# SpacewaIker/python-raytracer

Hardware: AMD Instinct MI355X
Metric: Mrays/sec + frame ms, TwoSpheresPlane 1920×1080 @1/2/4/8 GPUs (higher is better)
Workload: dtype fp32 vectors + fp64 scalars (reference numerics); 1 GPU; TwoSpheresPlane 1920x1080 1spp (primary + shadow rays); width=1920, height=1080, spp=1, parallelism=single GPU

## Files before the change

### python-raytracer_amd/csrc/rtx_api.hip

```cpp
#include <hip/hip_runtime.h>
#include <hip/hiprtc.h>

#include <algorithm>
#include <chrono>
#include <cmath>
#include <cstdio>
#include <cstring>
#include <dirent.h>
#include <fstream>
#include <functional>
#include <future>
#include <list>
#include <map>
#include <numeric>
#include <mutex>
#include <sstream>
#include <string>
#include <sys/stat.h>
#include <unistd.h>
#include <vector>

#include "../../include/rtx.h"
#include "rtx_kernels.h"
#include "rtx_bins.h"
// ... 19 lines not shown
    return code;
}

#define RTX_HIP(call)                                                                     \
    do {                                                                                  \
        hipError_t e_ = (call);                                                           \
        if (e_ != hipSuccess)                                                             \
            return fail(RTX_ERR_HIP, std::string(#call ": ") + hipGetErrorString(e_));    \
    } while (0)

enum Opt {
    OPT_SPLIT, OPT_SPLIT_BYTES, OPT_SPLIT_RATIO, OPT_BINS, OPT_HEAVY_TILES, OPT_LENS_BINS, OPT_LGRID, OPT_DSGRID, OPT_DSGRID_MIN,
    OPT_SELF_SKIP, OPT_TILE_SCHED, OPT_XCD_MAP, OPT_TILE_BLOCK, OPT_PRIM_ORIGIN, OPT_SPP, OPT_SPP_MIN, OPT_JIT, OPT_JIT_BAKE, OPT_JIT_EXT,
    OPT_JIT_DUMP, OPT_JIT_IDLE_BAKED, OPT_JIT_DISK_BAKED, OPT_JIT_CACHE, OPT_JIT_FLAGS, OPT_JIT_ILP, OPT_JIT_ASYNC,
    OPT_DEV_BINS, OPT_CHUNK_MODE, OPT_BIN_LDS, OPT_JIT_CSG, OPT_CSG_RAYS, OPT_CSG_SHADE, OPT_SETUP_LOG, OPT_SHADOW_BINS,
    OPT_UNIFORM_HIT, OPT_RAY_TABLE, OPT_RAY_TABLE_MAX_MB, OPT_COUNT
};
struct OptDef {
    const char* name;
    double dflt;
    bool str;
};
constexpr OptDef kOpts[OPT_COUNT] = {
    {"split", 1, false},
    {"split_bytes", 2147483648.0, false},
    {"split_ratio", -1, false},
    {"bins", 1, false},
    {"heavy_tiles", 1, false},
    {"lens_bins", 1, false},
    {"lgrid", 1, false},
    {"dsgrid", 1, false},
// ... 14 lines not shown
    {"jit_cache", 0, true},
    {"jit_flags", 0, true},
    {"jit_ilp", 1, false},
    {"jit_async", 1, false},
    {"dev_bins", 1, false},
    {"chunk_mode", 3, false},
    {"bin_lds", 0, false},
    {"jit_csg", 1, false},
    {"csg_rays", 3, false},
    {"csg_shade", 0, false},
    {"setup_log", 0, false},
    {"shadow_bins", 1, false},
    {"uniform_hit", 1, false},
    {"ray_table", 1, false},
    {"ray_table_max_mb", 64, false},
};
struct OptVal {
    double v;
    std::string s;
};
std::mutex g_opt_mu;
OptVal* opt_table() {
    static OptVal* t = [] {
        static OptVal vals[OPT_COUNT];
        for (int i = 0; i < OPT_COUNT; ++i) {
            vals[i].v = kOpts[i].dflt;
            std::string env = "RTX_";
            for (const char* c = kOpts[i].name; *c; ++c) env += (char)toupper((unsigned char)*c);
            if (const char* e = getenv(env.c_str())) {
                if (kOpts[i].str) vals[i].s = e;
// ... 938 lines not shown
    std::stable_sort(order.begin(), order.end(), [&](int32_t a2, int32_t b2) { return fz[a2] < fz[b2]; });
    for (int32_t f : order)
        for (int32_t by = rects[f].r0; by <= rects[f].r1; ++by)
            for (int32_t bx = rects[f].c0; bx <= rects[f].c1; ++bx) faces[fill[(size_t)by * nbx + bx]++] = f;
    zmin.resize(faces.size());
    for (size_t q = 0; q < faces.size(); ++q) {
        float z = (float)fz[faces[q]];
        if ((double)z > fz[faces[q]]) z = std::nextafter(z, -INFINITY);
        zmin[q] = z;
    }
    mesh_bins = 1;
    return true;
}

struct SbV { double x, y, z; };
struct SbPlane { SbV n; double num, dperp0; };
struct SbObj { SbV lo, hi, ctr; double r; uint32_t bit; int32_t sphere, always, pad; };
struct SbLight { SbV v; int32_t point, pad; };
constexpr int kSbPlanes = 8, kSbObjs = 32, kSbLights = 8, kSbSeen = 8, kSbPoints = 4 * kSbPlanes + 8 * kSbSeen;
struct SbScene {
    SbV o, cu, cv, cw;
    double d, dx, dy, margin, omag;
    int32_t W, H, bins_x, bins_y, NL, n_plane, n_obs, pad;
    uint32_t all_bits, always_bits;
    SbPlane planes[kSbPlanes];
    SbObj obs[kSbObjs];
    SbLight lights[kSbLights];
};
RTX_HD SbV sb_sub(SbV a, SbV b) { return SbV{a.x - b.x, a.y - b.y, a.z - b.z}; }
RTX_HD double sb_dot(SbV a, SbV b) { return a.x * b.x + a.y * b.y + a.z * b.z; }
RTX_HD SbV sb_axpy(SbV a, double t, SbV b) { return SbV{a.x + t * b.x, a.y + t * b.y, a.z + t * b.z}; }
RTX_HD bool sb_fin(SbV a) { return __builtin_isfinite(a.x) && __builtin_isfinite(a.y) && __builtin_isfinite(a.z); }

RTX_HD bool sb_separated(const SbV* P, int n, const SbLight& Lt, const SbObj& q, double grow) {
    SbV x = P[0];
    for (int it = 0; it < 12; ++it) {
        SbV u = sb_sub(q.ctr, x);
// ... 29 lines not shown
        if (q.sphere) {
            omin = sb_dot(u, q.ctr) - (q.r + grow) * sqrt(uu);
        } else {
            omin = fmin(u.x * (q.lo.x - grow), u.x * (q.hi.x + grow)) + fmin(u.y * (q.lo.y - grow), u.y * (q.hi.y + grow)) +
                   fmin(u.z * (q.lo.z - grow), u.z * (q.hi.z + grow));
        }
        if (m < omin - 1e-9 * (fabs(m) + fabs(omin) + 1.0)) return true;
        const SbV w = sb_sub(s, x);
        const double ww = sb_dot(w, w), t = ww > 0.0 ? sb_dot(u, w) / ww : 0.0;
        if (!(t > 1e-12)) return false;
        x = sb_axpy(x, fmin(t, 1.0), w);
    }
    return false;
}

RTX_HD void sb_bin(const SbScene& S, const float* xs, const float* ys, const uint32_t* objmask, int32_t bx, int32_t by,
                   uint32_t* out) {
    for (int32_t l = 0; l < S.NL; ++l) out[l] = S.all_bits;
    const int32_t c0 = 8 * bx, c1 = (8 * bx + 8 < S.W ? 8 * bx + 8 : S.W) - 1;
    const int32_t r0 = 8 * by, r1 = (8 * by + 8 < S.H ? 8 * by + 8 : S.H) - 1;
    const double px = 2.0 * S.margin * S.dx, py = 2.0 * S.margin * S.dy;
    const double xl = (double)xs[c0] - px, xh = (double)xs[c1] + px;
    const double yl = (double)ys[S.H - 1 - r1] - py, yh = (double)ys[S.H - 1 - r0] + py;
    if (!(xl < xh && yl < yh)) return;
    SbV dir[4];
    for (int q = 0; q < 4; ++q) {
        const double x = (q & 1) ? xh : xl, y = (q & 2) ? yh : yl;
        const SbV d{x * S.cu.x + y * S.cv.x - S.d * S.cw.x, x * S.cu.y + y * S.cv.y - S.d * S.cw.y,
                    x * S.cu.z + y * S.cv.z - S.d * S.cw.z};
        const double dd = sqrt(sb_dot(d, d));
        if (!(dd > 0.0) || !__builtin_isfinite(dd)) return;
        dir[q] = SbV{d.x / dd, d.y / dd, d.z / dd};
    }
    SbV P[kSbPoints];
    int np = 0;
    double rho = 0.0;
    for (int32_t k = 0; k < S.n_plane; ++k) {
        const SbPlane& pl = S.planes[k];
        const double sg = pl.num > 0.0 ? 1.0 : -1.0;
        double g[4], gmin = INFINITY, gmax = -INFINITY;
        for (int q = 0; q < 4; ++q) {
            g[q] = sg * sb_dot(dir[q], pl.n);
            gmin = fmin(gmin, g[q]);
            gmax = fmax(gmax, g[q]);
        }
        if (gmax <= 0.0) continue;
        if (!(gmin >= 1e-3)) return;
        double mp = 0.0;
        for (int q = 0; q < 4; ++q) {
            const SbV p = sb_axpy(S.o, fabs(pl.num) / g[q], dir[q]);
            P[np++] = p;
            mp = fmax(mp, fabs(p.x) + fabs(p.y) + fabs(p.z));
        }
        rho = fmax(rho, (pl.dperp0 + 0x1p-18 * mp) / gmin + 0x1p-20 * mp);
    }
    const uint32_t om = objmask[(int64_t)by * S.bins_x + bx];
    if (om) {
        const SbV mid{dir[0].x + dir[1].x + dir[2].x + dir[3].x, dir[0].y + dir[1].y + dir[2].y + dir[3].y,
                      dir[0].z + dir[1].z + dir[2].z + dir[3].z};
        const double mm = sqrt(sb_dot(mid, mid));
        double cosa = 1.0;
        for (int q = 0; q < 4; ++q) cosa = fmin(cosa, sb_dot(mid, dir[q]) / mm);
        if (!(cosa > 0.1)) return;
        int seen = 0;
        for (int32_t i = 0; i < S.n_obs; ++i) {
            const SbObj& q = S.obs[i];
            if (!(om & q.bit)) continue;
            if (++seen > kSbSeen) return;
            const double ov[3] = {S.o.x, S.o.y, S.o.z}, lo[3] = {q.lo.x, q.lo.y, q.lo.z}, hi[3] = {q.hi.x, q.hi.y, q.hi.z};
            double n2 = 0.0, f2 = 0.0;
            for (int a = 0; a < 3; ++a) {
// ... 17 lines not shown
        if (np == 0) {
            out[l] = S.always_bits;
            continue;
        }
        uint32_t m = S.all_bits;
        for (int32_t i = 0; i < S.n_obs; ++i) {
            const SbObj& q = S.obs[i];
            if (q.always || (om & q.bit)) continue;
            double dmax = 0.0;
            for (int j = 0; j < np; ++j) dmax = fmax(dmax, sb_dot(sb_sub(P[j], q.ctr), sb_sub(P[j], q.ctr)));
            const double grow = S.margin * ((q.sphere ? 0x1p-8 : 0x1p-10) * (sqrt(dmax) + q.r) + rho);
            if (sb_separated(P, np, S.lights[l], q, grow)) m &= ~q.bit;
        }
        out[l] = m | S.always_bits;
    }
}

__global__ __launch_bounds__(64) void k_shadow_bins(const SbScene* __restrict__ S, const float* __restrict__ xs,
                                                     const float* __restrict__ ys, const uint32_t* __restrict__ objmask,
                                                     uint32_t* __restrict__ out) {
    const int32_t b = (int32_t)(blockIdx.x * 64 + threadIdx.x);
    if (b >= S->bins_x * S->bins_y) return;
    sb_bin(*S, xs, ys, objmask, b % S->bins_x, b / S->bins_x, out + (int64_t)b * S->NL);
}

bool shadow_bins_scene(const HostScene& H, const rtx_camera_desc* c, int32_t bins_x, double margin, SbScene& S) {
    auto ldd = [](const float* p) { return SbV{(double)p[0], (double)p[1], (double)p[2]}; };
    auto amax = [](SbV a) { return std::max(std::fabs(a.x), std::max(std::fabs(a.y), std::fabs(a.z))); };
    std::memset(&S, 0, sizeof(S));
    const int32_t NL = (int32_t)H.lights.size();
    if (NL < 1 || NL > kSbLights || H.n_mesh > 0 || H.has_ext || H.n_sphere + H.n_box == 0 || H.n_sphere + H.n_box > kSbObjs ||
        H.n_plane > kSbPlanes)
        return false;
    if (c->ncols < 2 || c->height < 2 || bins_x != (c->ncols + 7) / 8) return false;
    const bool pinhole = c->n_dof == 1 && c->n_aa == 1 && c->jitter == RTX_JITTER_OFF &&
                         c->dof_origins[0] == c->position[0] && c->dof_origins[1] == c->position[1] &&
                         c->dof_origins[2] == c->position[2];
    if (!pinhole) return false;
    S.W = c->ncols; S.H = c->height; S.bins_x = bins_x; S.bins_y = (c->height + 7) / 8; S.NL = NL;
    S.o = ldd(c->aa_origins); S.cu = ldd(c->u); S.cv = ldd(c->v); S.cw = ldd(c->w);
    S.d = c->d;
    S.margin = margin;
    S.omag = amax(S.o);
    if (!sb_fin(S.o) || !sb_fin(S.cu) || !sb_fin(S.cv) || !sb_fin(S.cw) || !std::isfinite(S.d)) return false;
    for (int32_t i = 1; i < S.W; ++i) S.dx = std::max(S.dx, (double)c->xs[i] - (double)c->xs[i - 1]);
    for (int32_t j = 1; j < S.H; ++j) S.dy = std::max(S.dy, (double)c->ys[j] - (double)c->ys[j - 1]);
    if (!(S.dx > 0.0) || !(S.dy > 0.0) || !std::isfinite(S.dx + S.dy)) return false;
    double tlo = INFINITY, thi = -INFINITY;
    for (float t : camera_times(c)) {
        tlo = std::min(tlo, (double)t);
        thi = std::max(thi, (double)t);
    }
    S.n_plane = H.n_plane;
    for (int32_t k = 0; k < H.n_plane; ++k) {
        const DObj& ob = H.objs[k];
        if (ob.has_speed) return false;
        const SbV n = ldd(ob.b), p0 = ldd(ob.a);
        const double nn = std::sqrt(sb_dot(n, n));
        if (!sb_fin(n) || !sb_fin(p0) || !(nn > 0.0)) return false;
        SbPlane& pl = S.planes[k];
        pl.n = SbV{n.x / nn, n.y / nn, n.z / nn};
        pl.num = sb_dot(sb_sub(p0, S.o), pl.n);
        const double n1 = (std::fabs(n.x) + std::fabs(n.y) + std::fabs(n.z)) / nn;
        pl.dperp0 = 0x1p-19 * n1 * (std::fabs(p0.x) + std::fabs(p0.y) + std::fabs(p0.z) + std::fabs(S.o.x) + std::fabs(S.o.y) + std::fabs(S.o.z));
        if (!(std::fabs(pl.num) > 1e-9 * (1.0 + amax(p0) + S.omag))) return false;
    }
    S.n_obs = H.n_sphere + H.n_box;
    for (int32_t k = 0; k < S.n_obs; ++k) {
        const DObj& ob = H.objs[H.n_plane + k];
        SbObj& q = S.obs[k];
        q.sphere = k < H.n_sphere;
        const int32_t kk = q.sphere ? k : k - H.n_sphere;
        q.bit = 1u << ((q.sphere ? 0 : 16) + (kk & 15));
        q.always = ob.has_speed || (q.sphere ? H.n_sphere : H.n_box) > 16;
        double lo[3], hi[3];
        if (q.sphere) {
// ... 33 lines not shown
        if (!sb_fin(S.lights[l].v) || (!S.lights[l].point && !(sb_dot(S.lights[l].v, S.lights[l].v) > 0.0))) return false;
    }
    return true;
}

[[maybe_unused]] bool shadow_bins(const HostScene& H, const rtx_camera_desc* c, const std::vector<uint32_t>& objmask,
                                  int32_t bins_x, std::vector<uint32_t>& smask, double margin = 1.0) {
    smask.clear();
    SbScene S;
    if (!shadow_bins_scene(H, c, bins_x, margin, S) || objmask.size() < (size_t)S.bins_x * S.bins_y) return false;
    smask.assign((size_t)S.bins_x * S.bins_y * S.NL, S.all_bits);
    for (int32_t by = 0; by < S.bins_y; ++by)
        for (int32_t bx = 0; bx < S.bins_x; ++bx)
            sb_bin(S, c->xs, c->ys, objmask.data(), bx, by, smask.data() + ((size_t)by * S.bins_x + bx) * S.NL);
    return true;
}

bool light_grids(const HostScene& H, std::vector<DLGrid>& grids, std::vector<int32_t>& start,
                 std::vector<int32_t>& faces, std::vector<float>& d2) {
    grids.assign(H.lights.size(), DLGrid{});
    start.clear();
    faces.clear();
    d2.clear();
    if (H.n_mesh != 1) return false;
    const DObj& m = H.objs[H.n_plane + H.n_sphere + H.n_box];
    const int32_t F = m.tri_count;
    if (F < 1) return false;
    auto vert = [&](int32_t f, int k, int a) -> double {
        const DTri& T = H.tris[m.tri_begin + f];
        return k == 0 ? T.v0[a] : k == 1 ? T.v1[a] : T.v2[a];
// ... 517 lines not shown
            if (g.p) memcpy(h + g.off, g.p, g.n);
            else if (!g.dev) memset(h + g.off, 0, std::max<size_t>(g.n, 4));
        }
    }
};

struct CamTables {
    using DevFaces = std::function<int(int32_t bins_x, std::vector<int32_t>& start, int32_t* npairs, int32_t* mesh_bins)>;

    bool replay = false;
    bool pself = false;
    bool bins = false;
    bool dev_faces = false;
    bool heavy = false;
    bool sbins = false;
    bool tsched = false;
    bool po = false;
    bool rays = false;
    bool rays_dev = false;

    std::vector<float> times;
    CamStage st;
    std::vector<DBox> boxes;
    std::vector<float> pself_lim;
    std::vector<DSGrid> grids;
    std::vector<int32_t> ident, bstart, bfaces;
    std::vector<float> bz;
    std::vector<uint32_t> bmask, brmask;
    std::vector<int32_t> bheavy;
    std::vector<int2> hitems;
    SbScene sbs;
    int32_t bins_x = 0, mesh_bins = 0, dev_pairs = 0;
    int64_t tiles = 0;

    size_t host_bytes = 0;
    size_t o_xs = 0, o_ys = 0, o_dof = 0, o_aa = 0, o_times = 0, o_noise = 0, o_bounds = 0, o_pself = 0, o_dsg = 0;
    size_t o_bstart = 0, o_bfaces = 0, o_bz = 0, o_bmask = 0, o_bheavy = 0, o_hitems = 0, o_mhits = 0, o_sbs = 0;
    size_t o_bshadow = 0, o_tperm = 0, o_ttime = 0, o_kp = 0, o_rays = 0, rays_bytes = 0;

    int build(const HostScene& H, const rtx_camera_desc* c, std::vector<float> times_, const TimeTables& tr,
              const DevFaces& dev1, SetupLog& slog, bool on_device = false) {
        const size_t nsamp = (size_t)c->n_dof * c->n_aa;
        const double omax = camera_origin_bound(c);
        times = std::move(times_);
        o_xs = st.put(c->xs, sizeof(float) * c->ncols);
        o_ys = st.put(c->ys, sizeof(float) * c->height);
        o_dof = st.put(c->dof_origins, sizeof(float) * 3 * c->n_dof);
        o_aa = st.put(c->aa_origins, sizeof(float) * 3 * nsamp);
        o_times = st.put(times);
        replay = c->jitter == RTX_JITTER_REPLAY;
        if (replay) o_noise = st.put(c->noise, sizeof(float) * 3 * (size_t)c->ncols * c->height * nsamp);
        slog.mark("tables", st.size());
// ... 25 lines not shown
            o_bstart = st.put(bstart);
            if (!dev_faces) {
                o_bfaces = st.put(bfaces);
                o_bz = st.put(bz);
            }
            o_bmask = st.put(bmask);
        }
        heavy = bins && mesh_bins && !H.has_ext && opt_on(OPT_HEAVY_TILES) && heavy_chunks(bstart, bheavy, hitems);
        if (heavy) {
            o_bheavy = st.put(bheavy);
            o_hitems = st.put(hitems);
        }
        sbins = bins && opt_on(OPT_SHADOW_BINS) && (!H.has_secondary || opt(OPT_SHADOW_BINS) >= 2) && !H.has_mesh &&
                !H.has_ext && shadow_bins_scene(H, c, bins_x, 1.0, sbs);
        if (sbins) o_sbs = st.put(&sbs, sizeof(sbs));
        slog.mark("bins", st.size());
        tsched = opt_on(OPT_TILE_SCHED) && !H.has_ext && (H.has_secondary || H.has_mesh);
        int64_t nw = 0;
        if (tsched) {
            const int64_t wpb = kBlock<false> / 64;
            tiles = (int64_t)((c->ncols + 7) / 8) * ((c->height + 7) / 8);
            nw = (tiles + wpb - 1) / wpb * wpb;
            ident.resize((size_t)nw);
            std::iota(ident.begin(), ident.end(), 0);
            o_tperm = st.put(ident);
        }
        o_kp = st.put(nullptr, sizeof(KParams));
        bool boxed = true;
        for (const DObj& o : H.objs) boxed = boxed && (o.type != RTX_MESH || o.face_cull);
        rays_bytes = sizeof(float) * 3 * (size_t)ray_table_slots(c->height, c->ncols);
        rays = opt_on(OPT_RAY_TABLE) && c->n_dof == 1 && c->n_aa == 1 && c->n_times == 1 &&
               c->jitter == RTX_JITTER_OFF && !H.has_ext && ((!H.has_secondary && boxed) || opt(OPT_RAY_TABLE) == 4.0) &&
               (double)rays_bytes <= opt(OPT_RAY_TABLE_MAX_MB) * 1048576.0;
        rays_dev = rays && on_device;
        if (rays && !rays_dev) o_rays = st.put(nullptr, rays_bytes);
        host_bytes = st.size();
        if (dev_faces) {
            o_bfaces = st.put(nullptr, sizeof(int32_t) * dev_pairs, true);
            o_bz = st.put(nullptr, sizeof(float) * dev_pairs, true);
        }
        if (heavy) o_mhits = st.put(nullptr, sizeof(uint2) * 64 * hitems.size(), true);
        if (sbins) o_bshadow = st.put(nullptr, sizeof(uint32_t) * (size_t)sbs.bins_x * sbs.bins_y * sbs.NL, true);
        if (tsched) o_ttime = st.put(nullptr, sizeof(uint32_t) * nw, true);
        if (rays_dev) o_rays = st.put(nullptr, rays_bytes, true);
        slog.mark("tile schedule", st.size());
        po = c->n_dof == 1 && c->n_aa == 1 && c->jitter == RTX_JITTER_OFF && !any_moving(H) && !H.has_ext &&
             !H.has_secondary && H.n_plane <= 4 && H.n_sphere <= 16 && opt_on(OPT_PRIM_ORIGIN);
        return RTX_OK;
    }

    void bind(KParams& k, char* D, const HostScene& H, const rtx_camera_desc* c, const TimeTables& tr) const {
        k.xs = (cptr<float>)(D + o_xs);
        k.ys = (cptr<float>)(D + o_ys);
        k.dof_o = (cptr<float>)(D + o_dof);
        k.aa_o = (cptr<float>)(D + o_aa);
        k.times = (cptr<float>)(D + o_times);
        k.noise = replay ? (cptr<float>)(D + o_noise) : nullptr;
        if (!H.nodes.empty()) bind_boxes(k.S, (const DBox*)(D + o_bounds), H.nodes.size());
        if (pself) k.S.plane_self = (cptr<float>)(D + o_pself);
        if (tr.grids_on) bind_dir_grids(k.S, (const DSGrid*)(D + o_dsg), tr.cells_at());
        if (bins) {
            k.S.bin_objmask = (cptr<uint32_t>)(D + o_bmask);
            k.S.bin_rootmask = (cptr<uint32_t>)(D + o_bmask) + brmask.size();
            k.S.mesh_bins = mesh_bins;
            k.S.bin_start = (cptr<int32_t>)(D + o_bstart);
            k.S.bin_faces = (cptr<int32_t>)(D + o_bfaces);
            k.S.bin_zmin = (cptr<float>)(D + o_bz);
            k.S.bins_x = bins_x;
            k.S.bins_on = 1;
        }
        if (sbins) k.S.bin_shadow = (cptr<uint32_t>)(D + o_bshadow);
        if (heavy) {
            k.S.bin_heavy = (cptr<int32_t>)(D + o_bheavy);
            k.S.mesh_hits = reinterpret_cast<const uint2*>(D + o_mhits);
        }
        if (po) {
            const f3 o = mk(c->aa_origins[0], c->aa_origins[1], c->aa_origins[2]);
            int oi = 0;
            for (int q = 0; q < H.n_plane; ++q, ++oi) {
                const DObj& ob = H.objs[oi];
                k.po_pnum[q] = dot(sub(moved(ob, ob.a, 0.0f), o), ld3(ob.b));
            }
            for (int q = 0; q < H.n_sphere; ++q, ++oi) {
                const DObj& ob = H.objs[oi];
                const f3 oc = sub(o, moved(ob, ob.a, 0.0f));
                k.po_soc[q][0] = oc.x; k.po_soc[q][1] = oc.y; k.po_soc[q][2] = oc.z;
// ... 218 lines not shown
    if (!spp && !ext && kp.tile_time != nullptr) opts.push_back("-DRTX_TILE_SCHED=1");
    if (!spp && !ext && kp.po_valid) opts.push_back("-DRTX_PRIM_ORIGIN=1");
    if (!spp && opt_on(OPT_XCD_MAP)) opts.push_back("-DRTX_XCD_MAP=1");
    if (out8) opts.push_back("-DRTX_OUT8=1");
    if (sec && v.n_mats <= 64) opts.push_back("-DRTX_FRAME_MATBITS=6");
    if (sec && !mesh && !ext) {
        opts.push_back("-DRTX_DEFER_TIES=1");
        opts.push_back("-DRTX_HIT_T64_INLINE=1");
        opts.push_back("-DRTX_TIE_CALL=1");
        opts.push_back("-DRTX_FRAME_LDS_LEVELS=6");
        opts.push_back("-URTX_LB_WAVES");
        opts.push_back("-DRTX_LB_WAVES(MESH,SEC)=7");
    }
    opts.push_back(std::string("-DRTX_PRIMARY_BINS=") + (kp.S.bins_on ? "1" : "0"));
    if (kp.S.bins_on && kp.S.bin_shadow != nullptr) opts.push_back("-DRTX_SHADOW_BINS=1");
    if (!spp && !ext && kp.ray_dirs != nullptr && kp.n_dof * kp.n_aa * kp.n_times == 1 && kp.jitter == RTX_JITTER_OFF) {
        opts.push_back("-DRTX_RAY_TABLE=1");
        opts.push_back("-DRTX_FB_GLOBAL=1");
    }
    if (mesh && !ext && kp.S.bins_on && kp.S.mesh_bins && opt_on(OPT_BIN_LDS)) opts.push_back("-DRTX_BIN_LDS=1");
    opts.push_back(std::string("-DRTX_LIGHT_GRIDS=") + (v.lgrid_on ? "1" : "0"));
    opts.push_back(std::string("-DRTX_DIR_GRIDS=") + (kp.S.dsg_on ? "1" : "0"));
    for (const char* m : kLibMacros) opts.push_back(m);
    if (!ext && jit_block(mesh, sec, ext, spp) != kBlock<false>) {
        opts.push_back("-URTX_BLOCK_FLAT");
        opts.push_back("-DRTX_BLOCK_FLAT=" + std::to_string(jit_block(mesh, sec, ext, spp)));
    }
    if (!sec && !ext && (!mesh || fc_mode == 1)) {
        opts.push_back("-URTX_LB_WAVES");
        opts.push_back("-DRTX_LB_WAVES(MESH,SEC)=6");
// ... 789 lines not shown
#if defined(RTX_WAVE_LOG)
    if (const char* e = getenv("RTX_WAVE_LOG_PTR"))
        k.wave_log = reinterpret_cast<unsigned long long*>((uintptr_t)strtoull(e, nullptr, 0));
#endif
    if ((rc = pinned_reserve(s, T.host_bytes))) return rc;
    T.st.write(s->h_cam);
    memcpy(s->h_cam + T.o_kp, &k, sizeof(KParams));
    for (const auto& r : T.st.runs())
        if ((rc = pinned_upload(s, D + r.first, r.second - r.first, r.first))) return rc;
    slog.mark("upload");
    if (T.sbins) {
        const int32_t nbin = T.sbs.bins_x * T.sbs.bins_y;
        hipLaunchKernelGGL(k_shadow_bins, dim3((unsigned)((nbin + 63) / 64)), dim3(64), 0, nullptr,
                           reinterpret_cast<const SbScene*>(D + T.o_sbs), reinterpret_cast<const float*>(D + T.o_xs),
                           reinterpret_cast<const float*>(D + T.o_ys), reinterpret_cast<const uint32_t*>(D + T.o_bmask),
                           reinterpret_cast<uint32_t*>(D + T.o_bshadow));
        RTX_HIP(hipGetLastError());
        RTX_HIP(hipStreamSynchronize(nullptr));
        slog.mark("shadow bins (device)");
    }
    if (T.rays) {
        const int64_t nslots = ray_table_slots(k.height, k.ncols);
        hipLaunchKernelGGL(k_ray_dirs, dim3((unsigned)((nslots + 255) / 256)), dim3(256), 0, nullptr,
                           reinterpret_cast<const KParams*>(D + T.o_kp), reinterpret_cast<float*>(D + T.o_rays), nslots);
        RTX_HIP(hipGetLastError());
        if (!s->rays_event) RTX_HIP(hipEventCreateWithFlags(&s->rays_event, hipEventDisableTiming));
        RTX_HIP(hipEventRecord(s->rays_event, nullptr));
        s->rays_pending = true;
        char step[64];
        snprintf(step, sizeof(step), "ray table (device) [%zu B]", T.rays_bytes);
        slog.mark(step);
// ... 413 lines not shown
        while (T > 1 && std::gcd(m, T) != 1) ++m;
        L.perm = (uint32_t)(T > 1 ? m % T : 1);
#else
        L.perm = 1;
#endif
        L.pix0 = 0;
        L.tperm = 0;
        L.tlog = 0;
        L.xcd = opt_on(OPT_XCD_MAP) ? 1 : 0;
        L.redo = RedoList{nullptr, nullptr, nullptr};
        L.xs = s->kp.xs;
        L.ys = s->kp.ys;
        L.bin_objmask = s->kp.S.bin_objmask;
        L.bin_shadow = s->kp.S.bin_shadow;
        L.ray_dirs = s->kp.ray_dirs;
    }
    auto heavy_pass = [&](bool tiles) -> int {
        if (s->heavy_n <= 0 || !tiles || s->has_ext) return RTX_OK;
        hipLaunchKernelGGL(k_mesh_chunks, dim3((unsigned)s->heavy_n), dim3(64), 0, st, kp, L,
                           s->d_heavy_items, s->heavy_n, s->d_mesh_hits, (int32_t)opt(OPT_CHUNK_MODE));
        RTX_HIP(hipGetLastError());
        return RTX_OK;
    };
    JitSlot& rs = s->resolved[(out8 ? 8 : 0) | (cnt ? 4 : 0) | (jit ? 2 : 0) | (spp_mode ? 1 : 0)];
    if (!rs.done) {
        rs.block = jit_block(s->has_mesh, s->has_secondary, s->has_ext, spp_mode);
        rs.xcd = opt_on(OPT_XCD_MAP);
        jit_render_kernel(s->device, s->view, s->kp, s->traits, s->has_mesh, s->has_secondary, s->has_ext, cnt, jit,
                          spp_mode, out8, s->jit_baked, rs);
        if (rs.pending && !opt_on(OPT_JIT_ASYNC) && !stream_capturing(st)) jit_poll(rs, true);
// ... 341 lines not shown
```

### python-raytracer_amd/csrc/rtx_kernels.h

```cpp
#pragma once

#include "rtx_trace.h"
#if defined(__HIPCC_RTC__)
#include "rtx.h"
#else
#include "../../include/rtx.h"
#endif

namespace rtx {

struct alignas(64) KParams {
    float pos[4], u[4], v[4], dw[4];
    float focal, divisor, jscale, inv_divisor;
    int32_t width, height, col0, ncols;
    float dof0[4], aa0[4];
    int32_t po_valid, pad_h0, pad_h1, pad_h2;
    float po_pnum[4];
    float po_sq[16];
    float po_soc[16][3];
    SceneView S;
    cptr<float> xs;
    cptr<float> ys;
    cptr<float> dof_o;
    cptr<float> aa_o;
// ... 176 lines not shown
        return S;
    }
#endif
#if defined(__HIP_DEVICE_COMPILE__)
    if (RTX_RELOAD_RECORDS && !X) {
        S.objs = opaque_uniform(S.objs);
        if (RTX_RELOAD_RECORDS > 1) {
            S.mats = opaque_uniform(S.mats);
            S.lights = opaque_uniform(S.lights);
        }
    }
#endif
    return S;
}

template <bool MESH, bool SEC, bool X, bool COUNT, bool JIT>
RTX_HD void render_pixel(const KParams& P, float* fb, int32_t row0, int32_t rr, int32_t cc, Tally& tl,
                         const FrameStack& fs, const HStack& hs, int32_t bin = -1, int32_t tb = 0,
                         const f3* tdir = nullptr) {
#ifdef RTX_FIXED_NCOLS
    const int32_t ncols = RTX_FIXED_NCOLS;
#else
    const int32_t ncols = P.ncols;
#endif
    if (RTX_PROBE(14)) {
        const int64_t p = (int64_t)rr * ncols + cc;
        put_channel(fb, 3 * p, 0.5f); put_channel(fb, 3 * p + 1, 0.25f); put_channel(fb, 3 * p + 2, 0.125f);
        return;
    }
    const int j = P.height - 1 - (row0 + rr);
    const int32_t blane = bin >= 0 ? (((row0 + rr) & 7) << 3) | (cc & 7) : -1;
#if defined(RTX_PRIM_ORIGIN) && RTX_PRIM_ORIGIN && defined(RTX_FIXED_COUNTS)
    OriginTerms prim;
#pragma unroll
    for (int k = 0; k < RTX_FIXED_NP; ++k) prim.pnum[k] = P.po_pnum[k];
#pragma unroll
    for (int k = 0; k < RTX_FIXED_NS; ++k) {
        prim.soc[k] = ld3(P.po_soc[k]);
        prim.sq[k] = P.po_sq[k];
    }
    const OriginTerms* primp = &prim;
#else
    const OriginTerms* primp = nullptr;
#endif
    f3 colour = mk(0.0f, 0.0f, 0.0f);
    f3 jr_odd = mk(0.0f, 0.0f, 0.0f);
// ... 136 lines not shown
    float* fb;
    unsigned long long* counters;
    int32_t row0, nrows;
    int32_t gphase, gstride;
    int64_t fstride;
    uint32_t perm;
    int32_t pix0;
    int32_t tperm;
    int32_t tlog;
    int32_t xcd;
    int32_t tbase, tstep;
    RedoList redo;
    cptr<float> xs, ys;
    cptr<uint32_t> bin_objmask, bin_shadow;
    cptr<float> ray_dirs;
};

__device__ __forceinline__ float* frame_fb(const Launch& L) {
    return reinterpret_cast<float*>(reinterpret_cast<char*>(L.fb) + (int64_t)blockIdx.y * L.fstride);
}

#ifndef RTX_SEQUENCE
#if defined(__HIPCC_RTC__)
#define RTX_SEQUENCE 0
#else
#define RTX_SEQUENCE 1
#endif
#endif

RTX_HD int32_t time_base(const Launch& L) {
// ... 189 lines not shown
        return ld3(tdirs + 3u * ray_slot(image_row(L, rq), px.c, ncols));
    };
    f3 tdir = mk(0.0f, 0.0f, 0.0f);
#if !RTX_TILE_SCHED
    const PixelRC px_early = pixel_rc<B>(ncols, 0, L.perm, L.xcd);
    tdir = table_dir(px_early);
#endif
    Q.xs = nullptr;
    Q.ys = nullptr;
#else
    Q.xs = L.xs;
    Q.ys = L.ys;
#endif
    Q.S.bin_objmask = L.bin_objmask;
    Q.S.bin_shadow = L.bin_shadow;
    if (!X) {
        pin_uniform(Q.pos[0], Q.pos[1], Q.pos[2], Q.focal);
        pin_uniform(Q.u[0], Q.u[1], Q.u[2], Q.dof0[0]);
        pin_uniform(Q.v[0], Q.v[1], Q.v[2], Q.dof0[1]);
        pin_uniform(Q.dw[0], Q.dw[1], Q.dw[2], Q.dof0[2]);
        pin_uniform(Q.aa0[0], Q.aa0[1], Q.aa0[2], Q.S.ambient[0]);
        pin_uniform(Q.height, Q.S.bins_x, Q.S.bins_on, Q.ncols);
#if !RTX_RAY_TABLE
        pin_uniform64(Q.xs, Q.ys);
#endif
        pin_uniform64(Q.S.bin_objmask, Q.S.bin_shadow);
    }
    float* fbp = frame_fb(L);
    int64_t fbw = L.fstride;
    if (!X) pin_uniform64(fbp, fbw);
// ... 16 lines not shown
#endif
    for (int sub = 0; sub < RTX_PPL; ++sub) {
#if RTX_TILE_SCHED && defined(__HIP_DEVICE_COMPILE__)
        const PixelRC px = pixel_rc<B>(ncols, sub, L.perm, L.xcd, L.tperm ? Pp->tile_perm : nullptr, &tile);
#elif RTX_WAVE_HEAD && RTX_RAY_TABLE
        const PixelRC px = px_early;
#else
        const PixelRC px = pixel_rc<B>(ncols, sub, L.perm, L.xcd);
#endif
#if RTX_WAVE_HEAD && RTX_RAY_TABLE && RTX_TILE_SCHED
        tdir = table_dir(px);
#endif
        const bool active = px.r < L.nrows && px.c < ncols;
        any_active = any_active || active;
        const int32_t bin = RTX_TILE == 1 ? primary_bin(P.S, image_row(L, px.r & ~7), px.c & ~7) : -1;
#if RTX_WAVE_HEAD && RTX_TILE == 1 && RTX_PRIMARY_BINS
        if (!X && bin >= 0) Q.S.tile_objmask = Q.S.bin_objmask[wave_uniform(bin)];
#endif
#if RTX_WAVE_HEAD && RTX_RAY_TABLE
        if (active)
            render_pixel<MESH, SEC, X, COUNT, JIT>(P, fbp, image_row(L, px.r) - px.r, px.r, px.c, tl, fs, hs, bin,
                                                   tb, &tdir);
#else
        if (active)
            render_pixel<MESH, SEC, X, COUNT, JIT>(P, fbp, image_row(L, px.r) - px.r, px.r, px.c, tl, fs, hs, bin,
                                                   tb);
#endif
    }
    flush_tally<COUNT>(tl, L.counters, any_active);
#if RTX_TILE_SCHED && defined(__HIP_DEVICE_COMPILE__)
    if (L.tlog && (threadIdx.x & 63) == 0 && tile < Pp->tile_n)
// ... 699 lines not shown
```

### python-raytracer_amd/csrc/rtx_trace.h

```cpp
#pragma once

#if !defined(__HIPCC_RTC__)
#include <hip/hip_runtime.h>
#include <stdint.h>
#else
using __hip_internal::int32_t;
using __hip_internal::int64_t;
using __hip_internal::uint8_t;
using __hip_internal::uint16_t;
using __hip_internal::uint32_t;
using __hip_internal::uint64_t;
#ifndef INFINITY
#define INFINITY __builtin_inff()
#endif
#endif

#define RTX_HD __host__ __device__ __forceinline__

#include "rtx_fastmath.h"

#if defined(__HIP_DEVICE_COMPILE__)
#define RTX_CONST __attribute__((address_space(4)))
#else
#define RTX_CONST
// ... 244 lines not shown
    cptr<uint32_t> bin_rootmask;
    int32_t bins_x, bins_on, mesh_bins, pad5;
    cptr<int32_t> bin_heavy;
    const uint2* mesh_hits;
    int32_t n_objs_all, n_mats, pad6, pad7;
    cptr<DLGrid> lgrid;
    cptr<int32_t> lg_start;
    cptr<int32_t> lg_faces;
    cptr<float> lg_d2;
    int32_t lgrid_on, pad8, pad9, pad10;
    cptr<DSGrid> dsgrid;
    cptr<DSCell> dsg_cells;
    int32_t dsg_on, pad11, pad12, pad13;
    cptr<float> plane_self;
    cptr<uint32_t> bin_shadow;
    uint32_t tile_objmask, pad14, pad15, pad16;
};

#ifndef RTX_WAVE_HEAD
#if defined(RTX_FIXED_SAMPLES) && defined(__HIP_DEVICE_COMPILE__)
#define RTX_WAVE_HEAD (RTX_FIXED_NDOF * RTX_FIXED_NAA * RTX_FIXED_NTIMES == 1)
#else
#define RTX_WAVE_HEAD 0
#endif
#endif

#ifndef RTX_SHADOW_BINS
#ifdef RTX_FIXED_COUNTS
#define RTX_SHADOW_BINS 0
#else
#define RTX_SHADOW_BINS 1
#endif
// ... 2288 lines not shown
constexpr int kUniformHitMax = 4;
RTX_HD DMat select_mat(bool second, const DMat& a, const DMat& b) {
    constexpr int kWords = 18;
    static_assert(__builtin_offsetof(DMat, hardness) + sizeof(double) == 4 * kWords, "DMat's fields are 18 words");
    uint32_t wa[kWords], wb[kWords], wm[kWords];
    __builtin_memcpy(wa, &a, sizeof(wa));
    __builtin_memcpy(wb, &b, sizeof(wb));
    const uint32_t mask = second ? ~0u : 0u;
    for (int i = 0; i < kWords; ++i) wm[i] = wa[i] ^ ((wa[i] ^ wb[i]) & mask);
    DMat m = a;
    __builtin_memcpy(&m, wm, sizeof(wm));
    return m;
}
template <bool MESH, bool COUNT, int K>
RTX_HD f3 shade_uniform(const SceneView& S, const Hit& h, const HHit& hh, f3 o, f3 d, float time, Tally& tl,
                        const HStack& hs, int32_t bin) {
    const Surface sf = resolve_hit<MESH, false, K>(S, h, hh, o, d, time);
    const DObj ob = RTX_OBJ(S, K);
    const DMat m0 = RTX_MAT(S, ob.mat0);
    const DMat m = (ob.type != OBJ_PLANE || ob.nmat == 1) ? m0 : select_mat(sf.mat == ob.mat1, m0, RTX_MAT(S, ob.mat1));
    return regular_lighting<MESH, false, COUNT>(S, d, sf.position, sf.normal, m, ld3(m.diffuse), time, tl, hs, -1, K, bin);
}

template <bool MESH, bool SEC, bool X, bool COUNT>
RTX_HD f3 cast_ray(const SceneView& S, f3 o, f3 d, float time, Tally& tl, const FrameStack& fs, const HStack& hs,
                   int32_t bin = -1, const OriginTerms* prim = nullptr, int32_t blane = -1) {
    int nfr = 0;
    uint64_t fmats = 0;
    f3 deep[kMaxDepth - kFrameLds > 0 ? kMaxDepth - kFrameLds : 1];
    int32_t deep_mat[kMaxDepth - kFrameLds > 0 ? kMaxDepth - kFrameLds : 1];
    f3 tail = mk(0.0f, 0.0f, 0.0f);
    bool in_shape = false;
    for (int level = 0; level < (SEC ? kMaxDepth : 1); ++level) {
        if (COUNT) tl.cast[level]++;
        if (RTX_PROBE(8)) { tail = d; break; }
        HHit hh;
// ... 102 lines not shown
```

Baseline: 126,900 Mrays/s.

## Classify 8x8 tiles as sky/plane/unshadowed and fast-path unshadowed plane tiles

Extends the shadow-bin pass so it also records a per-tile class (sky, plane-only, plane with conservatively proven unshadowed lights) alongside the object mask in a packed uint2 record. The JIT kernel gets a RTX_TILE_CLASS path that loads this record wave-uniformly and, for unshadowed plane tiles, computes the plane hit analytically and shades with occlusion skipped. This removes closest-hit traversal and shadow-ray tests for the floor regions. It adds a wider per-tile load and a divergent code path, and correctness depends on the conservative bounds.

```diff
diff --git a/python-raytracer_amd/csrc/rtx_api.hip b/python-raytracer_amd/csrc/rtx_api.hip
--- a/python-raytracer_amd/csrc/rtx_api.hip
+++ b/python-raytracer_amd/csrc/rtx_api.hip
@@ -57,7 +57,7 @@
     OPT_SELF_SKIP, OPT_TILE_SCHED, OPT_XCD_MAP, OPT_TILE_BLOCK, OPT_PRIM_ORIGIN, OPT_SPP, OPT_SPP_MIN, OPT_JIT, OPT_JIT_BAKE, OPT_JIT_EXT,
     OPT_JIT_DUMP, OPT_JIT_IDLE_BAKED, OPT_JIT_DISK_BAKED, OPT_JIT_CACHE, OPT_JIT_FLAGS, OPT_JIT_ILP, OPT_JIT_ASYNC,
     OPT_DEV_BINS, OPT_CHUNK_MODE, OPT_BIN_LDS, OPT_JIT_CSG, OPT_CSG_RAYS, OPT_CSG_SHADE, OPT_SETUP_LOG, OPT_SHADOW_BINS,
-    OPT_UNIFORM_HIT, OPT_RAY_TABLE, OPT_RAY_TABLE_MAX_MB, OPT_COUNT
+    OPT_UNIFORM_HIT, OPT_RAY_TABLE, OPT_RAY_TABLE_MAX_MB, OPT_TILE_CLASS, OPT_COUNT
 };
 struct OptDef {
     const char* name;
@@ -102,6 +102,7 @@
     {"uniform_hit", 1, false},
     {"ray_table", 1, false},
     {"ray_table_max_mb", 64, false},
+    {"tile_class", 1, false},
 };
 struct OptVal {
     double v;
@@ -1070,13 +1071,14 @@
 }
 
 struct SbV { double x, y, z; };
-struct SbPlane { SbV n; double num, dperp0; };
+struct SbPlane { SbV n; double num, dperp0, nn; };
 struct SbObj { SbV lo, hi, ctr; double r; uint32_t bit; int32_t sphere, always, pad; };
 struct SbLight { SbV v; int32_t point, pad; };
 constexpr int kSbPlanes = 8, kSbObjs = 32, kSbLights = 8, kSbSeen = 8, kSbPoints = 4 * kSbPlanes + 8 * kSbSeen;
 struct SbScene {
     SbV o, cu, cv, cw;
     double d, dx, dy, margin, omag;
+    double cls_rho;
     int32_t W, H, bins_x, bins_y, NL, n_plane, n_obs, pad;
     uint32_t all_bits, always_bits;
     SbPlane planes[kSbPlanes];
@@ -1136,8 +1138,17 @@
     return false;
 }
 
-RTX_HD void sb_bin(const SbScene& S, const float* xs, const float* ys, const uint32_t* objmask, int32_t bx, int32_t by,
-                   uint32_t* out) {
+struct SbClass {
+    bool sky, plane, done;
+    double pmax;
+};
+
+RTX_HD void sb_bin_words(const SbScene& S, const float* xs, const float* ys, uint32_t om, int32_t bx, int32_t by,
+                         uint32_t* out, SbClass& cls) {
+    cls.sky = om == 0u;
+    cls.plane = om == 0u && S.n_plane == 1;
+    cls.done = false;
+    cls.pmax = INFINITY;
     for (int32_t l = 0; l < S.NL; ++l) out[l] = S.all_bits;
     const int32_t c0 = 8 * bx, c1 = (8 * bx + 8 < S.W ? 8 * bx + 8 : S.W) - 1;
     const int32_t r0 = 8 * by, r1 = (8 * by + 8 < S.H ? 8 * by + 8 : S.H) - 1;
@@ -1166,17 +1177,26 @@
             gmin = fmin(gmin, g[q]);
             gmax = fmax(gmax, g[q]);
         }
-        if (gmax <= 0.0) continue;
+        const bool num_sure = fabs(pl.num) > pl.dperp0;
+        if (gmax <= 0.0) {
+            cls.sky = cls.sky && gmax <= -1e-3 && num_sure;
+            cls.plane = false;
+            continue;
+        }
+        cls.sky = false;
         if (!(gmin >= 1e-3)) return;
-        double mp = 0.0;
+        double mp = 0.0, mi = 0.0;
         for (int q = 0; q < 4; ++q) {
             const SbV p = sb_axpy(S.o, fabs(pl.num) / g[q], dir[q]);
             P[np++] = p;
             mp = fmax(mp, fabs(p.x) + fabs(p.y) + fabs(p.z));
-        }
-        rho = fmax(rho, (pl.dperp0 + 0x1p-18 * mp) / gmin + 0x1p-20 * mp);
-    }
-    const uint32_t om = objmask[(int64_t)by * S.bins_x + bx];
+            mi = fmax(mi, fmax(fabs(p.x), fmax(fabs(p.y), fabs(p.z))));
+        }
+        const double rk = (pl.dperp0 + 0x1p-18 * mp) / gmin + 0x1p-20 * mp;
+        rho = fmax(rho, rk);
+        cls.plane = cls.plane && num_sure && gmin * pl.nn >= 2e-4 && mp < 1e30;
+        cls.pmax = mi + S.margin * S.cls_rho * (rk + 0x1p-22 * (mi + S.omag));
+    }
     if (om) {
         const SbV mid{dir[0].x + dir[1].x + dir[2].x + dir[3].x, dir[0].y + dir[1].y + dir[2].y + dir[3].y,
                       dir[0].z + dir[1].z + dir[2].z + dir[3].z};
@@ -1224,14 +1244,34 @@
         }
         out[l] = m | S.always_bits;
     }
+    cls.done = true;
+}
+
+RTX_HD void sb_bin(const SbScene& S, const float* xs, const float* ys, const uint32_t* objmask, int32_t bx, int32_t by,
+                   uint32_t* out, uint2* rec = nullptr, const float* pself = nullptr) {
+    const uint32_t om = objmask[(int64_t)by * S.bins_x + bx];
+    SbClass c;
+    sb_bin_words(S, xs, ys, om, bx, by, out, c);
+    if (rec == nullptr) return;
+    uint32_t w = 0u;
+    if (c.done && c.sky) w = kTileSky;
+    if (c.done && c.plane) {
+        w = kTilePlane;
+        bool free_ = pself != nullptr;
+        for (int32_t l = 0; l < S.NL && free_; ++l)
+            free_ = out[l] == 0u && pself[4 * l] != -1.0f && c.pmax <= (double)pself[4 * l];
+        if (free_) w |= kTileUnshadowed;
+    }
+    *rec = make_uint2(om, w);
 }
 
 __global__ __launch_bounds__(64) void k_shadow_bins(const SbScene* __restrict__ S, const float* __restrict__ xs,
                                                      const float* __restrict__ ys, const uint32_t* __restrict__ objmask,
-                                                     uint32_t* __restrict__ out) {
+                                                     uint32_t* __restrict__ out, uint2* __restrict__ rec,
+                                                     const float* __restrict__ pself) {
     const int32_t b = (int32_t)(blockIdx.x * 64 + threadIdx.x);
     if (b >= S->bins_x * S->bins_y) return;
-    sb_bin(*S, xs, ys, objmask, b % S->bins_x, b / S->bins_x, out + (int64_t)b * S->NL);
+    sb_bin(*S, xs, ys, objmask, b % S->bins_x, b / S->bins_x, out + (int64_t)b * S->NL, rec ? rec + b : nullptr, pself);
 }
 
 bool shadow_bins_scene(const HostScene& H, const rtx_camera_desc* c, int32_t bins_x, double margin, SbScene& S) {
@@ -1251,6 +1291,7 @@
     S.o = ldd(c->aa_origins); S.cu = ldd(c->u); S.cv = ldd(c->v); S.cw = ldd(c->w);
     S.d = c->d;
     S.margin = margin;
+    S.cls_rho = 1.0;
     S.omag = amax(S.o);
     if (!sb_fin(S.o) || !sb_fin(S.cu) || !sb_fin(S.cv) || !sb_fin(S.cw) || !std::isfinite(S.d)) return false;
     for (int32_t i = 1; i < S.W; ++i) S.dx = std::max(S.dx, (double)c->xs[i] - (double)c->xs[i - 1]);
@@ -1270,6 +1311,7 @@
         if (!sb_fin(n) || !sb_fin(p0) || !(nn > 0.0)) return false;
         SbPlane& pl = S.planes[k];
         pl.n = SbV{n.x / nn, n.y / nn, n.z / nn};
+        pl.nn = nn;
         pl.num = sb_dot(sb_sub(p0, S.o), pl.n);
         const double n1 = (std::fabs(n.x) + std::fabs(n.y) + std::fabs(n.z)) / nn;
         pl.dperp0 = 0x1p-19 * n1 * (std::fabs(p0.x) + std::fabs(p0.y) + std::fabs(p0.z) + std::fabs(S.o.x) + std::fabs(S.o.y) + std::fabs(S.o.z));
@@ -1333,6 +1375,13 @@
         for (int32_t bx = 0; bx < S.bins_x; ++bx)
             sb_bin(S, c->xs, c->ys, objmask.data(), bx, by, smask.data() + ((size_t)by * S.bins_x + bx) * S.NL);
     return true;
+}
+
+[[maybe_unused]] void tile_classes(const SbScene& S, const float* xs, const float* ys, const uint32_t* objmask,
+                                   const float* pself, uint2* rec) {
+    uint32_t words[kSbLights];
+    for (int32_t by = 0; by < S.bins_y; ++by)
+        for (int32_t bx = 0; bx < S.bins_x; ++bx) sb_bin(S, xs, ys, objmask, bx, by, words, rec + (size_t)by * S.bins_x + bx, pself);
 }
 
 bool light_grids(const HostScene& H, std::vector<DLGrid>& grids, std::vector<int32_t>& start,
@@ -1880,6 +1929,8 @@
     bool dev_faces = false;
     bool heavy = false;
     bool sbins = false;
+    bool tclass = false;
+    bool tclass_dev = false;
     bool tsched = false;
     bool po = false;
     bool rays = false;
@@ -1902,6 +1953,7 @@
     size_t host_bytes = 0;
     size_t o_xs = 0, o_ys = 0, o_dof = 0, o_aa = 0, o_times = 0, o_noise = 0, o_bounds = 0, o_pself = 0, o_dsg = 0;
     size_t o_bstart = 0, o_bfaces = 0, o_bz = 0, o_bmask = 0, o_bheavy = 0, o_hitems = 0, o_mhits = 0, o_sbs = 0;
+    size_t o_bclass = 0;
     size_t o_bshadow = 0, o_tperm = 0, o_ttime = 0, o_kp = 0, o_rays = 0, rays_bytes = 0;
 
     int build(const HostScene& H, const rtx_camera_desc* c, std::vector<float> times_, const TimeTables& tr,
@@ -1957,6 +2009,9 @@
         sbins = bins && opt_on(OPT_SHADOW_BINS) && (!H.has_secondary || opt(OPT_SHADOW_BINS) >= 2) && !H.has_mesh &&
                 !H.has_ext && shadow_bins_scene(H, c, bins_x, 1.0, sbs);
         if (sbins) o_sbs = st.put(&sbs, sizeof(sbs));
+        tclass = sbins && opt_on(OPT_TILE_CLASS) && !H.has_secondary && c->n_times == 1;
+        tclass_dev = tclass && on_device;
+        if (tclass && !tclass_dev) o_bclass = st.put(nullptr, sizeof(uint2) * (size_t)sbs.bins_x * sbs.bins_y);
         slog.mark("bins", st.size());
         tsched = opt_on(OPT_TILE_SCHED) && !H.has_ext && (H.has_secondary || H.has_mesh);
         int64_t nw = 0;
@@ -1984,6 +2039,7 @@
         }
         if (heavy) o_mhits = st.put(nullptr, sizeof(uint2) * 64 * hitems.size(), true);
         if (sbins) o_bshadow = st.put(nullptr, sizeof(uint32_t) * (size_t)sbs.bins_x * sbs.bins_y * sbs.NL, true);
+        if (tclass_dev) o_bclass = st.put(nullptr, sizeof(uint2) * (size_t)sbs.bins_x * sbs.bins_y, true);
         if (tsched) o_ttime = st.put(nullptr, sizeof(uint32_t) * nw, true);
         if (rays_dev) o_rays = st.put(nullptr, rays_bytes, true);
         slog.mark("tile schedule", st.size());
@@ -2013,6 +2069,9 @@
             k.S.bins_on = 1;
         }
         if (sbins) k.S.bin_shadow = (cptr<uint32_t>)(D + o_bshadow);
+        if (tclass) k.S.bin_class = (cptr<uint2>)(D + o_bclass);
+        if (tclass && !tclass_dev)
+            tile_classes(sbs, c->xs, c->ys, bmask.data(), pself ? pself_lim.data() : nullptr, reinterpret_cast<uint2*>(D + o_bclass));
         if (heavy) {
             k.S.bin_heavy = (cptr<int32_t>)(D + o_bheavy);
             k.S.mesh_hits = reinterpret_cast<const uint2*>(D + o_mhits);
@@ -2261,6 +2320,9 @@
     }
     opts.push_back(std::string("-DRTX_PRIMARY_BINS=") + (kp.S.bins_on ? "1" : "0"));
     if (kp.S.bins_on && kp.S.bin_shadow != nullptr) opts.push_back("-DRTX_SHADOW_BINS=1");
+    if (!spp && !ext && !sec && !mesh && kp.S.bins_on && kp.S.bin_shadow != nullptr && kp.S.bin_class != nullptr &&
+        kp.n_dof * kp.n_aa * kp.n_times == 1 && opt_on(OPT_TILE_CLASS))
+        opts.push_back("-DRTX_TILE_CLASS=1");
     if (!spp && !ext && kp.ray_dirs != nullptr && kp.n_dof * kp.n_aa * kp.n_times == 1 && kp.jitter == RTX_JITTER_OFF) {
         opts.push_back("-DRTX_RAY_TABLE=1");
         opts.push_back("-DRTX_FB_GLOBAL=1");
@@ -3080,7 +3142,9 @@
         hipLaunchKernelGGL(k_shadow_bins, dim3((unsigned)((nbin + 63) / 64)), dim3(64), 0, nullptr,
                            reinterpret_cast<const SbScene*>(D + T.o_sbs), reinterpret_cast<const float*>(D + T.o_xs),
                            reinterpret_cast<const float*>(D + T.o_ys), reinterpret_cast<const uint32_t*>(D + T.o_bmask),
-                           reinterpret_cast<uint32_t*>(D + T.o_bshadow));
+                           reinterpret_cast<uint32_t*>(D + T.o_bshadow),
+                           T.tclass ? reinterpret_cast<uint2*>(D + T.o_bclass) : nullptr,
+                           T.pself ? reinterpret_cast<const float*>(D + T.o_pself) : nullptr);
         RTX_HIP(hipGetLastError());
         RTX_HIP(hipStreamSynchronize(nullptr));
         slog.mark("shadow bins (device)");
@@ -3524,6 +3588,7 @@
         L.bin_objmask = s->kp.S.bin_objmask;
         L.bin_shadow = s->kp.S.bin_shadow;
         L.ray_dirs = s->kp.ray_dirs;
+        L.bin_class = s->kp.S.bin_class;
     }
     auto heavy_pass = [&](bool tiles) -> int {
         if (s->heavy_n <= 0 || !tiles || s->has_ext) return RTX_OK;
diff --git a/python-raytracer_amd/csrc/rtx_kernels.h b/python-raytracer_amd/csrc/rtx_kernels.h
--- a/python-raytracer_amd/csrc/rtx_kernels.h
+++ b/python-raytracer_amd/csrc/rtx_kernels.h
@@ -214,6 +214,32 @@
     return S;
 }
 
+#ifndef RTX_TILE_CLASS
+#define RTX_TILE_CLASS 0
+#endif
+template <bool COUNT>
+RTX_HD void render_pixel_plane(const KParams& P, float* fb, int32_t ncols, int32_t rr, int32_t cc, f3 o, f3 d, float time,
+                               Tally& tl, const HStack& hs) {
+    const SceneView S = sample_scene<false>(P.S);
+    if (COUNT) tl.cast[0]++;
+    const DObj ob = S.objs[0];
+    const f3 n = ld3(ob.b);
+    const float denom = dot(d, n);
+#if defined(RTX_PRIM_ORIGIN) && RTX_PRIM_ORIGIN && defined(RTX_FIXED_COUNTS)
+    const float num = P.po_pnum[0];
+#else
+    const float num = dot(sub(moved(ob, ob.a, time), o), n);
+#endif
+    const Hit h{num / denom, 0, 0};
+    HHit hh;
+    const f3 tail = clamp01(shade_uniform<false, COUNT, 0>(S, h, hh, o, d, time, tl, hs, -1, 0));
+    const f3 colour = add(mk(0.0f, 0.0f, 0.0f), tail);
+    const int64_t p = (int64_t)rr * ncols + cc;
+    put_channel(fb, 3 * p, sample_mean(P, colour.x));
+    put_channel(fb, 3 * p + 1, sample_mean(P, colour.y));
+    put_channel(fb, 3 * p + 2, sample_mean(P, colour.z));
+}
+
 template <bool MESH, bool SEC, bool X, bool COUNT, bool JIT>
 RTX_HD void render_pixel(const KParams& P, float* fb, int32_t row0, int32_t rr, int32_t cc, Tally& tl,
                          const FrameStack& fs, const HStack& hs, int32_t bin = -1, int32_t tb = 0,
@@ -230,6 +256,17 @@
     }
     const int j = P.height - 1 - (row0 + rr);
     const int32_t blane = bin >= 0 ? (((row0 + rr) & 7) << 3) | (cc & 7) : -1;
+#if !defined(__HIP_DEVICE_COMPILE__)
+    if (!MESH && !SEC && !X && bin >= 0 && P.S.bin_class != nullptr && P.n_dof * P.n_aa * P.n_times == 1) {
+        const uint32_t cls = P.S.bin_class[bin].y;
+        if (cls & kTileUnshadowed) {
+            const f3 d = P.ray_dirs != nullptr ? ld3(P.ray_dirs + 3 * (int64_t)ray_slot(row0 + rr, cc, ncols))
+                                               : primary_dir(P, cc, j, 0);
+            render_pixel_plane<COUNT>(P, fb, ncols, rr, cc, sample_origin<false>(P, cc, j, 0, 0), d, P.times[tb], tl, hs);
+            return;
+        }
+    }
+#endif
 #if defined(RTX_PRIM_ORIGIN) && RTX_PRIM_ORIGIN && defined(RTX_FIXED_COUNTS)
     OriginTerms prim;
 #pragma unroll
@@ -396,6 +433,7 @@
     cptr<float> xs, ys;
     cptr<uint32_t> bin_objmask, bin_shadow;
     cptr<float> ray_dirs;
+    cptr<uint2> bin_class;
 };
 
 __device__ __forceinline__ float* frame_fb(const Launch& L) {
@@ -615,6 +653,12 @@
 #endif
     Q.S.bin_objmask = L.bin_objmask;
     Q.S.bin_shadow = L.bin_shadow;
+#if RTX_TILE_CLASS
+    static_assert(!MESH && !SEC && !X && RTX_TILE == 1 && RTX_PPL == 1, "tile classes: flat primary + shadow kernels");
+    cptr<uint2> bclass = L.bin_class;
+    int64_t bclass_pad = 0;
+    pin_uniform64(bclass, bclass_pad);
+#endif
     if (!X) {
         pin_uniform(Q.pos[0], Q.pos[1], Q.pos[2], Q.focal);
         pin_uniform(Q.u[0], Q.u[1], Q.u[2], Q.dof0[0]);
@@ -661,7 +705,30 @@
         const bool active = px.r < L.nrows && px.c < ncols;
         any_active = any_active || active;
         const int32_t bin = RTX_TILE == 1 ? primary_bin(P.S, image_row(L, px.r & ~7), px.c & ~7) : -1;
-#if RTX_WAVE_HEAD && RTX_TILE == 1 && RTX_PRIMARY_BINS
+#if RTX_TILE_CLASS && RTX_WAVE_HEAD && RTX_PRIMARY_BINS
+        uint64_t rec = reinterpret_cast<cptr<uint64_t>>(bclass)[wave_uniform(bin >= 0 ? bin : 0)];
+#if defined(__HIP_DEVICE_COMPILE__)
+        asm volatile("" : "+s"(rec));
+#endif
+        if (bin >= 0) {
+            const uint32_t cls = (uint32_t)(rec >> 32);
+            Q.S.tile_objmask = (uint32_t)rec;
+            if (cls & kTileUnshadowed) {
+                if (active) {
+                    const int32_t row0c = image_row(L, px.r) - px.r;
+#if RTX_RAY_TABLE
+                    const f3 dc = tdir;
+#else
+                    const f3 dc = primary_dir(P, px.c, P.height - 1 - (row0c + px.r), 0);
+#endif
+                    render_pixel_plane<COUNT>(P, fbp, ncols, px.r, px.c,
+                                              sample_origin<false>(P, px.c, P.height - 1 - (row0c + px.r), 0, 0), dc,
+                                              P.times[tb], tl, hs);
+                }
+                continue;
+            }
+        }
+#elif RTX_WAVE_HEAD && RTX_TILE == 1 && RTX_PRIMARY_BINS
         if (!X && bin >= 0) Q.S.tile_objmask = Q.S.bin_objmask[wave_uniform(bin)];
 #endif
 #if RTX_WAVE_HEAD && RTX_RAY_TABLE
diff --git a/python-raytracer_amd/csrc/rtx_trace.h b/python-raytracer_amd/csrc/rtx_trace.h
--- a/python-raytracer_amd/csrc/rtx_trace.h
+++ b/python-raytracer_amd/csrc/rtx_trace.h
@@ -282,8 +282,11 @@
     int32_t dsg_on, pad11, pad12, pad13;
     cptr<float> plane_self;
     cptr<uint32_t> bin_shadow;
-    uint32_t tile_objmask, pad14, pad15, pad16;
-};
+    uint32_t tile_objmask, pad14;
+    cptr<uint2> bin_class;
+};
+
+constexpr uint32_t kTileSky = 1u, kTilePlane = 2u, kTileUnshadowed = 4u;
 
 #ifndef RTX_WAVE_HEAD
 #if defined(RTX_FIXED_SAMPLES) && defined(__HIP_DEVICE_COMPILE__)
@@ -2602,12 +2605,13 @@
 }
 template <bool MESH, bool COUNT, int K>
 RTX_HD f3 shade_uniform(const SceneView& S, const Hit& h, const HHit& hh, f3 o, f3 d, float time, Tally& tl,
-                        const HStack& hs, int32_t bin) {
+                        const HStack& hs, int32_t bin, int64_t occ_mask = -1) {
     const Surface sf = resolve_hit<MESH, false, K>(S, h, hh, o, d, time);
     const DObj ob = RTX_OBJ(S, K);
     const DMat m0 = RTX_MAT(S, ob.mat0);
     const DMat m = (ob.type != OBJ_PLANE || ob.nmat == 1) ? m0 : select_mat(sf.mat == ob.mat1, m0, RTX_MAT(S, ob.mat1));
-    return regular_lighting<MESH, false, COUNT>(S, d, sf.position, sf.normal, m, ld3(m.diffuse), time, tl, hs, -1, K, bin);
+    return regular_lighting<MESH, false, COUNT>(S, d, sf.position, sf.normal, m, ld3(m.diffuse), time, tl, hs, occ_mask, K,
+                                                bin);
 }
 
 template <bool MESH, bool SEC, bool X, bool COUNT>
```

New measurement: 133,600 Mrays/s (median of 6 runs). 1.05x the previous value.
